# Alvin-Zeng/DRN

Hardware: AMD Instinct MI355X
Metric: clips/sec fwd+bwd (BxT=256x4096 C3D feats) (higher is better)
Workload: dtype bf16; 1 GPU; Charades-STA-shaped C3D features, T=256, D=4096, batch 32/GPU, stage-1 losses; step = fwd+bwd+grad all-reduce+clip(0.5)+Adam; global_batch=32, T=256, D=4096, parallelism=dp1

## Files before the change

drn_amd/csrc/lstm.hip:

```cpp
#include <type_traits>
#include "common.h"
#include "../../include/drn_hip.h"

#define LSTM_THREADS 256
#define MAX_BT 4

__device__ __forceinline__ float sigmoidf_(float x) { return 1.f / (1.f + expf(-x)); }

struct LstmFwdArgs {
  const float* xproj;
  const void* Whh[2];
  float* hseq;
  _Float16* hseq16;
  float* cseq;
  float* gates;
  float* out;
  float* hprev_t;
  float* qvec;
  const float* b_ih[2];
  const float* b_hh[2];
  const long long* lengths;
  int B, L, H, s;
};

// ... 17 lines not shown
#pragma unroll
    for (int g = 0; g < 4; ++g) {
      e_x[g] = A.xproj[(((long)t * B + bq) * 2 + dir) * 4 * H + g * H + e_j];
      e_bi[g] = A.b_ih[dir][g * H + e_j];
      e_bh[g] = A.b_hh[dir][g * H + e_j];
    }
    const long sp = ((long)(dir * (L + 1) + (s > 0 ? s : 1)) * B + bq) * H + e_j;
    e_cp = A.cseq[sp];
    e_hp = A.hseq[sp];
    e_len = A.lengths[bq];
    if (s == 0) { e_cp = 0.f; e_hp = 0.f; }
  }
  if (s > 0) {
    const int kq = H / 4;
    const int col = l & 15;
    const long wrow = (long)((col & 3) * H + j0 + (col >> 2)) * H;
    if constexpr (std::is_same<WT, float>::value) {
      const float* W = (const float*)A.Whh[dir];
      const int kc = (l >> 4) * 4;
      for (int k0 = w * kq; k0 < (w + 1) * kq; k0 += 16 * KU) {
        f32x4 a[KU][MT], b[KU];
#pragma unroll
        for (int u = 0; u < KU; ++u) {
          const int k = k0 + u * 16 + kc;
          b[u] = *(const f32x4*)(W + wrow + k);
#pragma unroll
          for (int mt = 0; mt < MT; ++mt) {
            const int bb = mt * 16 + col;
            a[u][mt] = *(const f32x4*)(hprev + (long)(bb < B ? bb : 0) * H + k);
            if (bb >= B) a[u][mt] = (f32x4){0.f, 0.f, 0.f, 0.f};
          }
        }
#pragma unroll
        for (int u = 0; u < KU; ++u)
#pragma unroll
          for (int e = 0; e < 4; ++e)
#pragma unroll
            for (int mt = 0; mt < MT; ++mt) acc[mt] = __builtin_amdgcn_mfma_f32_16x16x4f32(a[u][mt][e], b[u][e], acc[mt], 0, 0, 0);
      }
    } else if constexpr (std::is_same<WT, _Float16>::value) {
      typedef _Float16 f16x8 __attribute__((ext_vector_type(8)));
      const float* W = (const float*)A.Whh[dir];
      const _Float16* h16 = A.hseq16 + ((long)(dir * (L + 1) + s) * B) * H;
      const int kc = (l >> 4) * 8;
      for (int k0 = w * kq; k0 < (w + 1) * kq; k0 += 32 * KU) {
        f16x8 a[KU][MT];
        f32x4 blo[KU], bhi[KU];
#pragma unroll
        for (int u = 0; u < KU; ++u) {
          const int k = k0 + u * 32 + kc;
          blo[u] = *(const f32x4*)(W + wrow + k);
          bhi[u] = *(const f32x4*)(W + wrow + k + 4);
#pragma unroll
          for (int mt = 0; mt < MT; ++mt) {
            const int bb = mt * 16 + col;
            a[u][mt] = *(const f16x8*)(h16 + (long)(bb < B ? bb : 0) * H + k);
            if (bb >= B)
#pragma unroll
              for (int e = 0; e < 8; ++e) a[u][mt][e] = (_Float16)0.f;
          }
        }
#pragma unroll
        for (int u = 0; u < KU; ++u) {
          f16x8 bv;
#pragma unroll
          for (int e = 0; e < 4; ++e) { bv[e] = (_Float16)blo[u][e]; bv[4 + e] = (_Float16)bhi[u][e]; }
#pragma unroll
          for (int mt = 0; mt < MT; ++mt) acc[mt] = __builtin_amdgcn_mfma_f32_16x16x32_f16(a[u][mt], bv, acc[mt], 0, 0, 0);
        }
      }
    }
  }
#pragma unroll
  for (int mt = 0; mt < MT; ++mt)
#pragma unroll
    for (int r = 0; r < 4; ++r) red[w][mt][l][r] = acc[mt][r];
  __syncthreads();
  if (!e_own) return;
  {
    const int bb = e_bb, j = e_j;
    const int mt = bb >> 4, r16 = bb & 15, ln = (r16 >> 2) * 16 + (threadIdx.x & 3) * 4, rg = r16 & 3;
    float pre[4];
#pragma unroll
    for (int g = 0; g < 4; ++g) {
      const float v = red[0][mt][ln + g][rg] + red[1][mt][ln + g][rg] + red[2][mt][ln + g][rg] + red[3][mt][ln + g][rg];
      pre[g] = v + e_x[g] + e_bi[g] + e_bh[g];
    }
    const float ig = sigmoidf_(pre[0]), fg = sigmoidf_(pre[1]), gg = tanhf(pre[2]), og = sigmoidf_(pre[3]);
    const long st_new = ((long)(dir * (L + 1) + s + 1) * B + bb) * H + j;
    const float cp = e_cp, hp = e_hp;
    const float cn = fg * cp + ig * gg;
    const float hn = og * tanhf(cn);
    const bool valid = t < e_len;
    A.cseq[st_new] = valid ? cn : cp;
    A.hseq[st_new] = valid ? hn : hp;
    if (A.hseq16) A.hseq16[st_new] = (_Float16)(valid ? hn : hp);
    float* gs = A.gates + (((long)t * B + bb) * 2 + dir) * 4 * H + j;
    gs[0] = ig; gs[H] = fg; gs[2 * H] = gg; gs[3 * H] = og;
    A.hprev_t[(((long)t * B + bb) * 2 + dir) * H + j] = hp;
    A.out[((long)bb * L + t) * 2 * H + dir * H + j] = valid ? hn : 0.f;
    if (A.qvec) {
      float* qv = A.qvec + (long)bb * 4 * H + dir * H + j;
      if (t == 0) qv[0] = valid ? hn : 0.f;
      if (t == e_len - 1) qv[2 * H] = hn;
    }
  }
}

template <typename WT, int MT>
static void lstm_fwd_launch(const LstmFwdArgs& A, hipStream_t stream) {
  dim3 grid(A.H / 4, 2);
  const int per = std::is_same<WT, float>::value ? 16 : 32;
  const int it = A.H / 4 / per;
  if (it % 8 == 0 && std::is_same<WT, float>::value) lstm_step_fwd_kernel<WT, MT, 8><<<grid, LSTM_THREADS, 0, stream>>>(A);
  else if (it % 4 == 0) lstm_step_fwd_kernel<WT, MT, 4><<<grid, LSTM_THREADS, 0, stream>>>(A);
  else if (it % 2 == 0) lstm_step_fwd_kernel<WT, MT, 2><<<grid, LSTM_THREADS, 0, stream>>>(A);
  else lstm_step_fwd_kernel<WT, MT, 1><<<grid, LSTM_THREADS, 0, stream>>>(A);
}

extern "C" int drn_lstm_step_fwd(const float* xproj, const void* Whh_f, const void* Whh_r, int w_dtype, const float* b_ih_f,
                                 const float* b_hh_f, const float* b_ih_r, const float* b_hh_r, float* hseq, float* cseq, float* gates,
                                 float* out, float* hprev_t, float* qvec, void* hseq16, const int64_t* lengths, int B, int L, int H, int s,
                                 void* stream_) {
  drn_clear_status();
  hipStream_t stream = (hipStream_t)stream_;
  DRN_CHECK_ARG(xproj && Whh_f && Whh_r && b_ih_f && b_hh_f && b_ih_r && b_hh_r && hseq && cseq && gates && out && hprev_t && lengths,
                "drn_lstm_step_fwd: null pointer");
  DRN_CHECK_ARG(B > 0 && B <= 16 * MAX_BT && L > 0 && H % 64 == 0 && s >= 0 && s < L, "drn_lstm_step_fwd: need B<=64, H%%64==0");
  DRN_CHECK_ARG(w_dtype == DRN_F32, "drn_lstm_step_fwd: W_hh is fp32 (low precision enters through hseq16)");
  LstmFwdArgs A;
  DRN_CHECK_ARG(!hseq16 || (w_dtype == DRN_F32 && H % 128 == 0), "drn_lstm_step_fwd: the fp16 state copy goes with fp32 weights and H %% 128 == 0");
  A.hseq16 = (_Float16*)hseq16;
  A.xproj = xproj; A.Whh[0] = Whh_f; A.Whh[1] = Whh_r; A.hseq = hseq; A.cseq = cseq; A.gates = gates; A.out = out;
  A.hprev_t = hprev_t; A.qvec = qvec; A.b_ih[0] = b_ih_f; A.b_hh[0] = b_hh_f; A.b_ih[1] = b_ih_r; A.b_hh[1] = b_hh_r;
  A.lengths = (const long long*)lengths; A.B = B; A.L = L; A.H = H; A.s = s;
  const int mt = cdiv(B, 16);
  if (hseq16) {
    if (mt == 1) lstm_fwd_launch<_Float16, 1>(A, stream); else if (mt == 2) lstm_fwd_launch<_Float16, 2>(A, stream);
    else if (mt == 3) lstm_fwd_launch<_Float16, 3>(A, stream); else lstm_fwd_launch<_Float16, 4>(A, stream);
  } else {
    if (mt == 1) lstm_fwd_launch<float, 1>(A, stream); else if (mt == 2) lstm_fwd_launch<float, 2>(A, stream);
    else if (mt == 3) lstm_fwd_launch<float, 3>(A, stream); else lstm_fwd_launch<float, 4>(A, stream);
  }
  return drn_launch_status("drn_lstm_step_fwd");
}

struct LstmSeqArgs {
  LstmFwdArgs f;
  unsigned long long* xch;
  unsigned* counter;
};
static __device__ int g_lstm_seq_timeouts;

template <int MT, int KU>
__global__ __launch_bounds__(LSTM_THREADS) void lstm_seq_fwd_kernel(const LstmSeqArgs S) {
  typedef _Float16 f16x8 __attribute__((ext_vector_type(8)));
  __shared__ float red[4][MT][64][4];
  __shared__ unsigned s_launch;
  const LstmFwdArgs& A = S.f;
  const int w = threadIdx.x >> 6, l = threadIdx.x & 63;
  const int dir = blockIdx.y, j0 = blockIdx.x * 4;
  const int B = A.B, L = A.L, H = A.H;
  if (threadIdx.x == 0) s_launch = __hip_atomic_fetch_add(S.counter, 1u, __ATOMIC_RELAXED, __HIP_MEMORY_SCOPE_AGENT) / (gridDim.x * gridDim.y) + 1u;
  const int e_bb = threadIdx.x >> 2, e_j = j0 + (threadIdx.x & 3);
  const bool e_own = e_bb < B;
  const int bq = e_own ? e_bb : 0;
  float e_bi[4], e_bh[4];
#pragma unroll
  for (int g = 0; g < 4; ++g) {
    e_bi[g] = A.b_ih[dir][g * H + e_j];
    e_bh[g] = A.b_hh[dir][g * H + e_j];
  }
  const long long e_len = A.lengths[bq];
  float e_cp = 0.f, e_hp = 0.f;
  const int kq = H / 4, col = l & 15, kc = (l >> 4) * 8;
  const long wrow = (long)((col & 3) * H + j0 + (col >> 2)) * H;
  const float* W = (const float*)A.Whh[dir];
  __syncthreads();
  const unsigned long long tagm = (s_launch & 1u) ? 0x4000400040004000ull : 0ull;
  const long long t0 = wall_clock64();
  const bool w_resident = kq == 32 * KU;
  f16x8 wv[KU];
  if (w_resident) {
#pragma unroll
    for (int u = 0; u < KU; ++u) {
      const int k = w * kq + u * 32 + kc;
      const f32x4 lo = *(const f32x4*)(W + wrow + k), hi = *(const f32x4*)(W + wrow + k + 4);
#pragma unroll
      for (int e = 0; e < 4; ++e) { wv[u][e] = (_Float16)lo[e]; wv[u][4 + e] = (_Float16)hi[e]; }
    }
  }
  for (int s = 0; s < L; ++s) {
    const int t = dir == 0 ? s : L - 1 - s;
    float e_x[4];
#pragma unroll
    for (int g = 0; g < 4; ++g) e_x[g] = A.xproj[(((long)t * B + bq) * 2 + dir) * 4 * H + g * H + e_j];
    f32x4 acc[MT];
#pragma unroll
    for (int mt = 0; mt < MT; ++mt) acc[mt] = (f32x4){0.f, 0.f, 0.f, 0.f};
    if (s > 0) {
      const unsigned long long* hx = S.xch + ((long)(dir * L + s - 1) * B) * (H / 4);
      if (w == 0) {
        bool ready = false;
        for (;;) {
          if (!ready) {
            ready = true;
            for (int p = l; p < H / 4; p += 64)
              ready = ready && ((__hip_atomic_load(hx + p, __ATOMIC_RELAXED, __HIP_MEMORY_SCOPE_AGENT) & 0x4000400040004000ull) == tagm);
          }
          if (__builtin_amdgcn_ballot_w64(!ready) == 0) break;
          __builtin_amdgcn_s_sleep(4);
          if (wall_clock64() - t0 > 200000000LL) break;
        }
      }
      __syncthreads();
      for (int k0 = w * kq; k0 < (w + 1) * kq; k0 += 32 * KU) {
        unsigned long long alo[KU][MT], ahi[KU][MT];
        f32x4 blo[KU], bhi[KU];
#pragma unroll
        for (int u = 0; u < KU; ++u) {
          const int k = k0 + u * 32 + kc;
          if (!w_resident) {
            blo[u] = *(const f32x4*)(W + wrow + k);
            bhi[u] = *(const f32x4*)(W + wrow + k + 4);
          }
#pragma unroll
          for (int mt = 0; mt < MT; ++mt) {
            const int bb = mt * 16 + col;
            const unsigned long long* q = hx + (long)(bb < B ? bb : 0) * (H / 4) + (k >> 2);
            alo[u][mt] = __hip_atomic_load(q, __ATOMIC_RELAXED, __HIP_MEMORY_SCOPE_AGENT);
            ahi[u][mt] = __hip_atomic_load(q + 1, __ATOMIC_RELAXED, __HIP_MEMORY_SCOPE_AGENT);
          }
        }
#pragma unroll
        for (int u = 0; u < KU; ++u) {
          f16x8 bv;
          if (w_resident) bv = wv[u];
          else
#pragma unroll
            for (int e = 0; e < 4; ++e) { bv[e] = (_Float16)blo[u][e]; bv[4 + e] = (_Float16)bhi[u][e]; }
#pragma unroll
          for (int mt = 0; mt < MT; ++mt) {
            const int bb = mt * 16 + col;
            const unsigned long long* q = S.xch + ((long)(dir * L + s - 1) * B + (bb < B ? bb : 0)) * (H / 4) + ((k0 + u * 32 + kc) >> 2);
            while ((alo[u][mt] & 0x4000400040004000ull) != tagm || (ahi[u][mt] & 0x4000400040004000ull) != tagm) {
              __builtin_amdgcn_s_sleep(2);
              if (wall_clock64() - t0 > 200000000LL) {
                __hip_atomic_fetch_add(&g_lstm_seq_timeouts, 1, __ATOMIC_RELAXED, __HIP_MEMORY_SCOPE_AGENT);
                break;
              }
              alo[u][mt] = __hip_atomic_load(q, __ATOMIC_RELAXED, __HIP_MEMORY_SCOPE_AGENT);
              ahi[u][mt] = __hip_atomic_load(q + 1, __ATOMIC_RELAXED, __HIP_MEMORY_SCOPE_AGENT);
            }
            const unsigned long long lo = alo[u][mt] & ~0x4000400040004000ull, hi = ahi[u][mt] & ~0x4000400040004000ull;
            typedef unsigned long long u64x2 __attribute__((ext_vector_type(2)));
            f16x8 av = __builtin_bit_cast(f16x8, (u64x2){lo, hi});
            if (bb >= B)
#pragma unroll
              for (int e = 0; e < 8; ++e) av[e] = (_Float16)0.f;
            acc[mt] = __builtin_amdgcn_mfma_f32_16x16x32_f16(av, bv, acc[mt], 0, 0, 0);
          }
        }
      }
    }
#pragma unroll
    for (int mt = 0; mt < MT; ++mt)
#pragma unroll
      for (int r = 0; r < 4; ++r) red[w][mt][l][r] = acc[mt][r];
    __syncthreads();
    float h_new = 0.f;
    if (e_own) {
      const int bb = e_bb, j = e_j;
      const int mt = bb >> 4, r16 = bb & 15, ln = (r16 >> 2) * 16 + (threadIdx.x & 3) * 4, rg = r16 & 3;
      float pre[4];
#pragma unroll
      for (int g = 0; g < 4; ++g) {
        const float v = red[0][mt][ln + g][rg] + red[1][mt][ln + g][rg] + red[2][mt][ln + g][rg] + red[3][mt][ln + g][rg];
        pre[g] = v + e_x[g] + e_bi[g] + e_bh[g];
      }
      const float ig = sigmoidf_(pre[0]), fg = sigmoidf_(pre[1]), gg = tanhf(pre[2]), og = sigmoidf_(pre[3]);
      const long st_new = ((long)(dir * (L + 1) + s + 1) * B + bb) * H + j;
      const float cp = e_cp, hp = e_hp;
      const float cn = fg * cp + ig * gg;
      const float hn = og * tanhf(cn);
      const bool valid = t < e_len;
      e_cp = valid ? cn : cp;
      e_hp = valid ? hn : hp;
      h_new = e_hp;
      if (s + 1 < L) {
        const unsigned hb = (unsigned)__builtin_bit_cast(unsigned short, (_Float16)h_new);
        const unsigned h1 = (unsigned)__shfl_down((int)hb, 1, 64), h2 = (unsigned)__shfl_down((int)hb, 2, 64), h3 = (unsigned)__shfl_down((int)hb, 3, 64);
        if ((threadIdx.x & 3) == 0) {
          const unsigned long long word = ((unsigned long long)hb | ((unsigned long long)h1 << 16) | ((unsigned long long)h2 << 32) | ((unsigned long long)h3 << 48)) | tagm;
          __hip_atomic_store(S.xch + ((long)(dir * L + s) * B + e_bb) * (H / 4) + (j0 >> 2), word, __ATOMIC_RELAXED, __HIP_MEMORY_SCOPE_AGENT);
        }
      }
      A.cseq[st_new] = e_cp;
      A.hseq[st_new] = e_hp;
      float* gs = A.gates + (((long)t * B + bb) * 2 + dir) * 4 * H + j;
      gs[0] = ig; gs[H] = fg; gs[2 * H] = gg; gs[3 * H] = og;
      A.hprev_t[(((long)t * B + bb) * 2 + dir) * H + j] = hp;
      A.out[((long)bb * L + t) * 2 * H + dir * H + j] = valid ? hn : 0.f;
      if (A.qvec) {
        float* qv = A.qvec + (long)bb * 4 * H + dir * H + j;
        if (t == 0) qv[0] = valid ? hn : 0.f;
        if (t == e_len - 1) qv[2 * H] = hn;
      }
    }
    __syncthreads();
  }
}

static int lstm_seq_capacity(const void* kernel) {
  int dev = 0, per_cu = 0, cus = 0;
  if (hipGetDevice(&dev) != hipSuccess) return 0;
  if (hipDeviceGetAttribute(&cus, hipDeviceAttributeMultiprocessorCount, dev) != hipSuccess) return 0;
  if (hipOccupancyMaxActiveBlocksPerMultiprocessor(&per_cu, kernel, LSTM_THREADS, 0) != hipSuccess) return 0;
  hipFuncAttributes fa;
  if (hipFuncGetAttributes(&fa, kernel) != hipSuccess || fa.localSizeBytes > 0) return 0;
  return per_cu * cus;
}

extern "C" int64_t drn_lstm_seq_fwd_ws_bytes(int B, int L, int H) { return 64 + (int64_t)2 * L * B * (H / 4) * 8; }

extern "C" int drn_lstm_seq_fwd(const float* xproj, const void* Whh_f, const void* Whh_r, const float* b_ih_f, const float* b_hh_f,
                                const float* b_ih_r, const float* b_hh_r, float* hseq, float* cseq, float* gates, float* out, float* hprev_t,
                                float* qvec, void* xch_ws, int64_t ws_bytes, const int64_t* lengths, int B, int L, int H, void* stream_) {
  drn_clear_status();
  hipStream_t stream = (hipStream_t)stream_;
  DRN_CHECK_ARG(xproj && Whh_f && Whh_r && b_ih_f && b_hh_f && b_ih_r && b_hh_r && hseq && cseq && gates && out && hprev_t && lengths && xch_ws,
                "drn_lstm_seq_fwd: null pointer");
  DRN_CHECK_ARG(B > 0 && B <= 16 * MAX_BT && L > 0 && H % 128 == 0, "drn_lstm_seq_fwd: need B <= 64, H %% 128 == 0");
  DRN_CHECK_ARG(((uintptr_t)xch_ws & 63) == 0 && ws_bytes >= drn_lstm_seq_fwd_ws_bytes(B, L, H), "drn_lstm_seq_fwd: workspace too small or misaligned");
  LstmSeqArgs S;
  LstmFwdArgs& A = S.f;
  A.hseq16 = nullptr;
  A.xproj = xproj; A.Whh[0] = Whh_f; A.Whh[1] = Whh_r; A.hseq = hseq; A.cseq = cseq; A.gates = gates; A.out = out;
  A.hprev_t = hprev_t; A.qvec = qvec; A.b_ih[0] = b_ih_f; A.b_hh[0] = b_hh_f; A.b_ih[1] = b_ih_r; A.b_hh[1] = b_hh_r;
  A.lengths = (const long long*)lengths; A.B = B; A.L = L; A.H = H; A.s = 0;
  S.counter = (unsigned*)xch_ws;
  S.xch = (unsigned long long*)((char*)xch_ws + 64);
  const int mt = cdiv(B, 16), it = H / 4 / 32;
  const dim3 grid(H / 4, 2);
  const int total = (H / 4) * 2;
#define SEQ_CASE(MTV, KUV) do { \
    static int cap = 0; \
    if (!cap) cap = lstm_seq_capacity((const void*)lstm_seq_fwd_kernel<MTV, KUV>); \
    if (total > cap) { drn_set_error("drn_lstm_seq_fwd: %d workgroups exceed the %d the chip holds at once", total, cap); return DRN_ERR_UNSUPPORTED; } \
    lstm_seq_fwd_kernel<MTV, KUV><<<grid, LSTM_THREADS, 0, stream>>>(S); } while (0)
#define SEQ_MT(KUV) do { if (mt == 1) SEQ_CASE(1, KUV); else if (mt == 2) SEQ_CASE(2, KUV); else if (mt == 3) SEQ_CASE(3, KUV); else SEQ_CASE(4, KUV); } while (0)
  if (it % 4 == 0) SEQ_MT(4); else if (it % 2 == 0) SEQ_MT(2); else SEQ_MT(1);
#undef SEQ_MT
#undef SEQ_CASE
  return drn_launch_status("drn_lstm_seq_fwd");
}

extern "C" int drn_lstm_seq_fwd_timeouts(int reset) {
  int v = 0;
  if (hipMemcpyFromSymbol(&v, HIP_SYMBOL(g_lstm_seq_timeouts), sizeof(int)) != hipSuccess) return -1;
  if (reset && v) {
    const int z = 0;
    (void)hipMemcpyToSymbol(HIP_SYMBOL(g_lstm_seq_timeouts), &z, sizeof(int));
  }
  return v;
}

struct LstmBwdArgs {
  const float* dout;
  const float* gates;
  const float* cseq;
  const void* WhhT[2];
  float* dgates;
  float* dc;
  float* dh_pass;
  bf16_t* dgates16;
  const float* dqvec;
  const long long* lengths;
  int B, L, H, s;
};

struct LstmCellIn {
  float dout, dcn, ig, fg, gg, og, cn, cp;
  bool valid;
};
__device__ __forceinline__ LstmCellIn lstm_cell_bwd_load(const LstmBwdArgs& A, int dir, int bb, int j, int s) {
  const int B = A.B, L = A.L, H = A.H;
  const int t = dir == 0 ? s : L - 1 - s;
  LstmCellIn c;
  const long long len = A.lengths[bb];
  c.valid = t < len;
  const long sidx = ((long)dir * B + bb) * H + j;
  c.dout = A.dout[((long)bb * L + t) * 2 * H + dir * H + j];
  if (A.dqvec) {
    const float* dq = A.dqvec + (long)bb * 4 * H + dir * H + j;
    const float d0 = dq[0], d1 = dq[2 * H];
    if (t == 0) c.dout += d0;
    if (t == len - 1) c.dout += d1;
  }
  c.dcn = s == L - 1 ? 0.f : A.dc[sidx];
  const float* gs = A.gates + (((long)t * B + bb) * 2 + dir) * 4 * H + j;
  c.ig = gs[0]; c.fg = gs[H]; c.gg = gs[2 * H]; c.og = gs[3 * H];
  c.cn = A.cseq[((long)(dir * (L + 1) + s + 1) * B + bb) * H + j];
  c.cp = A.cseq[((long)(dir * (L + 1) + (s > 0 ? s : 1)) * B + bb) * H + j];
  if (s == 0) c.cp = 0.f;
  return c;
}
__device__ __forceinline__ void lstm_cell_bwd_apply(const LstmBwdArgs& A, const LstmCellIn& c, int dir, int bb, int j, int s, float dh_in) {
#pragma clang fp contract(off)
  const int B = A.B, L = A.L, H = A.H;
  const int t = dir == 0 ? s : L - 1 - s;
  const long sidx = ((long)dir * B + bb) * H + j;
  const long gidx = (((long)t * B + bb) * 2 + dir) * 4 * H + j;
  float* dg = A.dgates + gidx;
  const float dh = dh_in + (c.valid ? c.dout : 0.f);
  const float dcn = c.dcn;
  float d0 = 0.f, d1 = 0.f, d2 = 0.f, d3 = 0.f;
  if (c.valid) {
    const float ig = c.ig, fg = c.fg, gg = c.gg, og = c.og, cn = c.cn, cp = c.cp;
    const float tc = tanhf(cn);
    const float dcv = dcn + dh * og * (1.f - tc * tc);
    d0 = dcv * gg * ig * (1.f - ig);
    d1 = dcv * cp * fg * (1.f - fg);
    d2 = dcv * ig * (1.f - gg * gg);
    d3 = dh * tc * og * (1.f - og);
    A.dc[sidx] = dcv * fg;
    A.dh_pass[sidx] = 0.f;
  } else {
    A.dc[sidx] = dcn;
    A.dh_pass[sidx] = dh;
  }
  dg[0] = d0; dg[H] = d1; dg[2 * H] = d2; dg[3 * H] = d3;
  if (A.dgates16) {
    bf16_t* dg16 = A.dgates16 + gidx;
    dg16[0] = (bf16_t)d0; dg16[H] = (bf16_t)d1; dg16[2 * H] = (bf16_t)d2; dg16[3 * H] = (bf16_t)d3;
  }
}
__device__ __forceinline__ void lstm_cell_bwd(const LstmBwdArgs& A, int dir, int bb, int j, int s, float dh_in) {
  const LstmCellIn c = lstm_cell_bwd_load(A, dir, bb, j, s);
  lstm_cell_bwd_apply(A, c, dir, bb, j, s, dh_in);
}

__global__ void lstm_bwd_first_kernel(const LstmBwdArgs A) {
  const int B = A.B, H = A.H;
  const int total = 2 * B * H;
  for (int idx = blockIdx.x * blockDim.x + threadIdx.x; idx < total; idx += gridDim.x * blockDim.x)
    lstm_cell_bwd(A, idx / (H * B), (idx / H) % B, idx % H, A.L - 1, 0.f);
}

template <typename WT, int KU>
__global__ __launch_bounds__(LSTM_THREADS) void lstm_step_bwd_kernel(const LstmBwdArgs A) {
  __shared__ float red[4][64][4];
  const int w = threadIdx.x >> 6, l = threadIdx.x & 63;
  const int dir = blockIdx.y, k0 = blockIdx.x * 16, bt = blockIdx.z;
  const int B = A.B, L = A.L, H = A.H, s = A.s;
  const int K = 4 * H, kq = K / 4;
  const int t = dir == 0 ? s : L - 1 - s;
  const float* dg = A.dgates + ((long)t * B * 2 + dir) * K;
  f32x4 acc = (f32x4){0.f, 0.f, 0.f, 0.f};
  const int row = l & 15;
  const int bb_a = bt * 16 + row;
  const int e_bb = bt * 16 + (l >> 4) * 4 + w, e_k = k0 + (l & 15);
  const bool e_own = e_bb < B;
  const LstmCellIn e_c = lstm_cell_bwd_load(A, dir, e_own ? e_bb : 0, e_k, s - 1);
  const float e_dhp = A.dh_pass[((long)dir * B + (e_own ? e_bb : 0)) * H + e_k];
  const float* arow = dg + (long)(bb_a < B ? bb_a : 0) * 2 * K;
  if constexpr (std::is_same<WT, float>::value) {
    const float* WT_ = (const float*)A.WhhT[dir];
    const int rc = (l >> 4) * 4;
    for (int r0 = w * kq; r0 < (w + 1) * kq; r0 += 16 * KU) {
      f32x4 a[KU], b[KU];
#pragma unroll
      for (int u = 0; u < KU; ++u) {
        const int r = r0 + u * 16 + rc;
        a[u] = *(const f32x4*)(arow + r);
        if (bb_a >= B) a[u] = (f32x4){0.f, 0.f, 0.f, 0.f};
        b[u] = *(const f32x4*)(WT_ + (long)(k0 + row) * K + r);
      }
#pragma unroll
      for (int u = 0; u < KU; ++u)
#pragma unroll
        for (int e = 0; e < 4; ++e) acc = __builtin_amdgcn_mfma_f32_16x16x4f32(a[u][e], b[u][e], acc, 0, 0, 0);
    }
  } else {
    const bf16_t* WT_ = (const bf16_t*)A.WhhT[dir];
    const int rc = (l >> 4) * 8;
    if (A.dgates16) {
      const bf16_t* arow16 = A.dgates16 + ((long)t * B * 2 + dir) * K + (long)(bb_a < B ? bb_a : 0) * 2 * K;
      for (int r0 = w * kq; r0 < (w + 1) * kq; r0 += 32 * KU) {
        bf16x8 a[KU], b[KU];
#pragma unroll
        for (int u = 0; u < KU; ++u) {
          const int r = r0 + u * 32 + rc;
          a[u] = *(const bf16x8*)(arow16 + r);
          if (bb_a >= B)
#pragma unroll
            for (int e = 0; e < 8; ++e) a[u][e] = (bf16_t)0.f;
          b[u] = *(const bf16x8*)(WT_ + (long)(k0 + row) * K + r);
        }
#pragma unroll
        for (int u = 0; u < KU; ++u) acc = __builtin_amdgcn_mfma_f32_16x16x32_bf16(a[u], b[u], acc, 0, 0, 0);
      }
    } else
// ... 69 lines not shown
```

drn_amd/trainer.py:

```python
import contextlib
import functools
import os

import torch

from . import functional as DF
import numpy as np

from .metrics import results_entries, PostProcessRunner, results_entry, recall_from_first_hits


def stage_plan(model, stage, lr):
    dead = set(id(p) for p in model.unused_parameters()) if hasattr(model, "unused_parameters") else set()
    if stage == 1:
        for name, p in model.named_parameters():
            if "iou_scores" in name or "mix_fc" in name:
                p.requires_grad = False
        return [p for p in model.parameters() if p.requires_grad and id(p) not in dead], lr, 10, "sum"
    if stage == 2:
        head = model.fcos.head
        return list(head.iou_scores.parameters()) + list(head.mix_fc.parameters()), lr / 100, None, "loss_iou"
    if stage == 3:
        return [p for p in model.parameters() if id(p) not in dead], lr / 10000, None, "sum"
    raise ValueError("stage must be 1, 2 or 3")
# ... 187 lines not shown
                        self.reducer.rearm()
                    slot.graph.replay()
                    if getattr(slot, "acc_outside", False):
                        self._accumulate(select_loss(slot.out, self.which), slot.feats.size(0))
                    if not whole:
                        self._exchange_and_update()
                    out = slot.out
                else:
                    slot.seen += 1
                    out = self._fwd_bwd(slot.args)
                    self._exchange_and_update()
        cur.wait_stream(self.stream)
        return out

    def train_step(self, args):
        self.model.train()
        if self.graph:
            return self._graph_step(args)
        if self.fused:
            self.reducer.zero()
        _, loss_dict = self.model(*args)
        DF.backward(select_loss(loss_dict, self.which))
        if self.fused:
            self.reducer.finish()
            self.opt.step()
        else:
            if self.world_size > 1:
                self._average_grads()
            if self.clip is not None:
                torch.nn.utils.clip_grad_norm_(self.model.parameters(), self.clip)
            self.opt.step()
            self.opt.zero_grad()
        return loss_dict

    def _average_grads(self):
        import torch.distributed as td
        grads = [p.grad for p in self.model.parameters() if p.grad is not None]
        if not grads:
            return
        flat = torch._utils._flatten_dense_tensors(grads)
        td.all_reduce(flat)
        flat.div_(self.world_size)
        for g, r in zip(grads, torch._utils._unflatten_dense_tensors(flat, grads)):
            g.copy_(r)

    def train_epoch(self, loader, epoch=None):
        sampler = getattr(loader, "sampler", None)
        if epoch is not None and hasattr(sampler, "set_epoch"):
            sampler.set_epoch(epoch)
        n = 0
        if getattr(self, "_loss_acc", None) is None:
            self._loss_acc = torch.zeros((), dtype=torch.float32, device=getattr(self, "device", "cpu"))
        if getattr(self, "graph", False) and getattr(self, "prefetch", False):
            it = iter(loader)
            nxt = self._prefetch(next(it, None))
            with torch.cuda.stream(self.stream):
                self._loss_acc.zero_()
            while nxt is not None:
                cur_b = nxt
                nxt = self._prefetch(next(it, None))
                bs = cur_b.batch_size if isinstance(cur_b, _Preloaded) else cur_b[2].size(0)
                self.train_step(cur_b)
                n += bs
            torch.cuda.current_stream().wait_stream(self.stream)
            return self._epoch_result(n)
        with torch.cuda.stream(self.stream) if self.graph else contextlib.nullcontext():
            self._loss_acc.zero_()
        for batch in loader:
            if self.graph:
                names, pse, feats, gt, tok, qlen, nprops, nframes = batch
                args = (tok, qlen, feats, pse, gt, nprops, nframes)
            else:
                _, args = to_device(batch, self.device)
            bs = args[2].size(0)
            ld = self.train_step(args)
            if not self.graph:
                self._accumulate(select_loss(ld, self.which), bs)
            n += bs
        if self.graph:
            torch.cuda.current_stream().wait_stream(self.stream)
        return self._epoch_result(n)

    def _epoch_result(self, n):
        mean = float(self._loss_acc) / max(n, 1) if n else 0.0
        if getattr(getattr(self, "device", None), "type", "cpu") == "cuda":
            from . import ops
            ops.check_watchdogs()
        return mean

    def _prefetch(self, batch):
        if batch is None:
            return None
        names, pse, feats, gt, tok, qlen, nprops, nframes = batch
        if all(t.is_cuda for t in (tok, qlen, feats, pse, gt)):
            return (tok, qlen, feats, pse, gt, nprops, nframes)
        slot = self._slot_for(tok, feats, pse, gt, alternate=True)
        if slot is None:
            return (tok, qlen, feats, pse, gt, nprops, nframes)
        if self._copy_stream is None:
            self._copy_stream = torch.cuda.Stream(device=self.device)
        cs = self._copy_stream
        cs.wait_stream(torch.cuda.current_stream())
        with torch.cuda.stream(cs):
            slot.load(tok, qlen, feats, pse, gt)
            ev = torch.cuda.Event()
            ev.record(cs)
        for t in (tok, qlen, feats, pse, gt):
            if t.is_cuda:
                t.record_stream(cs)
        return _Preloaded(slot, ev, int(feats.size(0)))

    @torch.no_grad()
    def evaluate(self, loader, id2word=None, iou_topk=None, with_results=True, group=None):
        self.model.eval()
        import torch.distributed as td
        multi = td.is_available() and td.is_initialized() and td.get_world_size(group) > 1
        if multi:
            from .dist import sync_model_state
            sync_model_state(self.model, src=0, group=group, buffers_only=True)
        iou_topk = iou_topk or {"iou": [0.5], "topk": [1, 5]}
        results, total, n, hits = {}, None, 0, []
        selector = getattr(getattr(self.model, "fcos", None), "box_selector_test", None)
        head = getattr(getattr(self.model, "fcos", None), "head", None)
        one_class = head is None or head.cls_logits.weight.shape[0] == 1
        fast = (not with_results) and selector is not None and self.device.type == "cuda" and one_class
        fast0 = fast
        ious_dev = torch.tensor([float(x) for x in iou_topk["iou"]], dtype=torch.float64, device=self.device) if fast else None
        if fast:
            selector.device_only = True
        try:
            for batch in loader:
                host_tok, host_qlen, host_gt = batch[4], batch[5], batch[3]
                names, args = to_device(batch, self.device)
                boxes, loss_dict = self.model(*args)
                bs = args[2].size(0)
                lsum = select_loss(loss_dict, self.which).detach().reshape(-1)[0].float() * bs
                total = lsum if total is None else total + lsum
                n += bs
                if fast and not isinstance(boxes, list):
                    from . import ops
                    hits.append(ops.eval_recall(boxes.det, boxes.scores, boxes.counts, args[4].contiguous(), ious_dev,
                                                max(iou_topk["topk"])))
                    continue
                if fast:
                    raise RuntimeError("Trainer.evaluate: the post-processor returned host records in device-only mode")
                tokens, qlen, gts = host_tok.cpu(), host_qlen.cpu(), host_gt.cpu().numpy()
                queries = [" ".join(id2word[int(t)] if id2word else str(int(t)) for t in tokens[i, :int(qlen[i])]) for i in range(bs)]
                for name, entry in zip(names, results_entries(queries, gts, boxes)):
                    results.setdefault(name, []).append(entry)
        finally:
            if fast:
                selector.device_only = False
        total = float(total) if total is not None else 0.0
        if fast0:
            fh = torch.cat(hits).cpu().numpy() if hits else np.zeros((0, len(iou_topk["iou"])), dtype=np.int32)
            if multi:
                parts = [None] * td.get_world_size(group)
                td.all_gather_object(parts, ("hits", fh, total, n), group=group)
                assert all(p[0] == "hits" for p in parts), "ranks disagree on the evaluation path"
                fh = np.concatenate([p[1] for p in parts])
                total, n = sum(p[2] for p in parts), sum(p[3] for p in parts)
            return total / max(n, 1), iou_topk["topk"], recall_from_first_hits(fh, iou_topk["iou"], iou_topk["topk"]), None
        if multi:
            parts = [None] * td.get_world_size(group)
            td.all_gather_object(parts, ("records", results, total, n), group=group)
            assert all(p[0] == "records" for p in parts), "ranks disagree on the evaluation path"
            parts = [p[1:] for p in parts]
            results = {}
            for part, _, _ in parts:
                for vid, items in part.items():
                    results.setdefault(vid, []).extend(items)
            total, n = sum(p[1] for p in parts), sum(p[2] for p in parts)
        topks, accs = PostProcessRunner(results).run_evaluate(iou_topk_dict=iou_topk, temporal_nms=True)
        return total / max(n, 1), topks, accs, results

    @torch.no_grad()
    def predict(self, loader, top_k=5, nms_overlap=0.45, share_videos=True, id2word=None, fused=False, graph=False):
        from .grounding import Grounder, group_by_video
        was_training = self.model.training
        self.model.eval()
        grounder = Grounder(self.model, top_k=top_k, nms_overlap=nms_overlap, fused=fused, graph=graph)
        out = {}
        try:
            for batch in loader:
                names, pse, feats, _, tok, qlen = batch[:6]
                mv = lambda t: t.to(self.device, non_blocking=True)
                vid = None
                if share_videos:
                    unique, vid = group_by_video(names)
                    if len(unique) < len(names):
                        first = torch.tensor([names.index(u) for u in unique], dtype=torch.int64)
                        feats, pse = feats.index_select(0, first.to(feats.device)), pse.index_select(0, first.to(pse.device))
                    else:
                        vid = None
                moments = grounder.ground(mv(tok), mv(qlen), mv(feats), mv(pse), vid).tolist()
                tokens, lens = tok.cpu(), qlen.cpu()
                for i, name in enumerate(names):
                    query = " ".join(id2word[int(t)] if id2word else str(int(t)) for t in tokens[i, :int(lens[i])])
                    out.setdefault(name, []).append({"query": query, "moments": moments[i]})
        finally:
            self.model.train(was_training)
        return out

    def fit(self, train_loader, test_loader, n_epoch=None, eval_freq=1, snapshot_pref=None, dataset="Charades", id2word=None,
            start_epoch=0, rank=0):
        n_epoch = self.default_epochs if self.default_epochs is not None else n_epoch
        best1 = best5 = 0.0
        history = []
        for epoch in range(start_epoch, n_epoch):
            train_loss = self.train_epoch(train_loader, epoch)
            rec = {"epoch": epoch, "train_loss": train_loss}
            if (epoch + 1) % eval_freq == 0 or epoch == n_epoch - 1:
                val_loss, topks, accs, _ = self.evaluate(test_loader, id2word, with_results=False)
                top1, top5 = accs[0] * 100, accs[1] * 100
                rec.update(val_loss=val_loss, top1=top1, top5=top5)
                state = {"epoch": epoch + 1, "state_dict": checkpoint_state_dict(self.model), "loss": val_loss, "top1": top1,
                         "top5": top5}
                if snapshot_pref is not None and rank == 0:
                    if top1 > best1:
                        save_checkpoint(state, snapshot_pref, dataset, epoch, top1, top5)
                    if top5 > best5:
                        save_checkpoint(state, snapshot_pref, dataset, epoch, top1, top5)
                best1, best5 = max(best1, top1), max(best5, top5)
            history.append(rec)
        return history


    def fit_train_only(self, train_loader, n_epoch, start_epoch=0):
        n_epoch = self.default_epochs if self.default_epochs is not None else n_epoch
        return [{"epoch": e, "train_loss": self.train_epoch(train_loader, e)} for e in range(start_epoch, n_epoch)]


def checkpoint_state_dict(model):
    DF.flush_bn_counters()
    return {"module." + k: v for k, v in model.state_dict().items()}


def checkpoint_name(snapshot_pref, dataset, epoch, top1, top5):
    return "{}/model_{}_epoch{}_top1_{:.3f}_top5_{:.3f}_model_best.pth.tar".format(snapshot_pref, dataset, epoch, top1, top5)


def save_checkpoint(state, snapshot_pref, dataset, epoch, top1, top5):
    os.makedirs(snapshot_pref, exist_ok=True)
    path = checkpoint_name(snapshot_pref, dataset, epoch, top1, top5)
    torch.save(state, path)
    return path


def load_checkpoint(model, path, map_location="cpu"):
    ckpt = torch.load(path, map_location=map_location)
    own = model.state_dict()
    picked = {}
    for k, v in ckpt["state_dict"].items():
        k = k[len("module."):] if k.startswith("module.") else k
        if k in own:
            picked[k] = v
    own.update(picked)
    model.load_state_dict(own)
    DF.bump_weights_epoch([DF.store_of(next(model.parameters()))])
    return ckpt.get("epoch", 0), sorted(picked)


def init_glove(model, glove_weights):
    if glove_weights and os.path.exists(glove_weights):
        model.query_encoder.embedding.weight.data.copy_(torch.load(glove_weights))
        DF.bump_weights_epoch([DF.store_of(model.query_encoder.embedding.weight)])
        return True
    return False
```

Before: 17490 clips/s.

## Widen LSTM sequence workgroups to 16 hidden units with LDS-resident recurrent weights

The persistent LSTM forward kernel now has each workgroup own 16 hidden units instead of 4, which cuts the grid by four. Each workgroup caches its slice of W_hh as fp16 in dynamic LDS, and each wave computes four MFMA N-tiles per h fragment, so every exchanged h load is reused four times. The wave-0 pre-spin barrier is removed, the gate math is spread across lanes via shuffles, and the next step's xproj is prefetched. The trade-off is a large LDS footprint per workgroup and fewer workgroups for the cross-block h exchange. The trainer also adds a watchdog check after evaluation.

```diff
diff --git a/drn_amd/csrc/lstm.hip b/drn_amd/csrc/lstm.hip
--- a/drn_amd/csrc/lstm.hip
+++ b/drn_amd/csrc/lstm.hip
@@ -193,170 +193,203 @@
 };
 static __device__ int g_lstm_seq_timeouts;
 
+#define SEQ_TAG 0x4000400040004000ull
+#define SEQ_TIMEOUT 200000000LL
+
+static inline size_t lstm_seq_lds_bytes(int H, int mt) { return (size_t)128 * H + (size_t)16384 * mt; }
+
 template <int MT, int KU>
 __global__ __launch_bounds__(LSTM_THREADS) void lstm_seq_fwd_kernel(const LstmSeqArgs S) {
   typedef _Float16 f16x8 __attribute__((ext_vector_type(8)));
-  __shared__ float red[4][MT][64][4];
+  extern __shared__ __attribute__((aligned(16))) char smem[];
   __shared__ unsigned s_launch;
   const LstmFwdArgs& A = S.f;
   const int w = threadIdx.x >> 6, l = threadIdx.x & 63;
-  const int dir = blockIdx.y, j0 = blockIdx.x * 4;
+  const int dir = blockIdx.y, j0 = blockIdx.x * 16;
   const int B = A.B, L = A.L, H = A.H;
+  const int kq = H / 4, ki = kq / 32;
+  f16x8* wf = (f16x8*)smem + (size_t)w * ki * 256;
+  float* red = (float*)(smem + (size_t)128 * H);
   if (threadIdx.x == 0) s_launch = __hip_atomic_fetch_add(S.counter, 1u, __ATOMIC_RELAXED, __HIP_MEMORY_SCOPE_AGENT) / (gridDim.x * gridDim.y) + 1u;
-  const int e_bb = threadIdx.x >> 2, e_j = j0 + (threadIdx.x & 3);
-  const bool e_own = e_bb < B;
-  const int bq = e_own ? e_bb : 0;
+  const int q = l & 3, cu = (l >> 2) & 3, rg = l >> 4;
+  const int e_j = j0 + w * 4 + cu;
   float e_bi[4], e_bh[4];
 #pragma unroll
   for (int g = 0; g < 4; ++g) {
     e_bi[g] = A.b_ih[dir][g * H + e_j];
     e_bh[g] = A.b_hh[dir][g * H + e_j];
   }
-  const long long e_len = A.lengths[bq];
-  float e_cp = 0.f, e_hp = 0.f;
-  const int kq = H / 4, col = l & 15, kc = (l >> 4) * 8;
-  const long wrow = (long)((col & 3) * H + j0 + (col >> 2)) * H;
-  const float* W = (const float*)A.Whh[dir];
+  int e_bb[MT], e_bq[MT];
+  long long e_len[MT];
+  float e_cp[MT], e_hp[MT], e_x[MT][4];
+#pragma unroll
+  for (int mt = 0; mt < MT; ++mt) {
+    e_bb[mt] = mt * 16 + rg * 4 + q;
+    e_bq[mt] = e_bb[mt] < B ? e_bb[mt] : 0;
+    e_len[mt] = A.lengths[e_bq[mt]];
+    e_cp[mt] = 0.f; e_hp[mt] = 0.f;
+    const int t = dir == 0 ? 0 : L - 1;
+#pragma unroll
+    for (int g = 0; g < 4; ++g) e_x[mt][g] = A.xproj[(((long)t * B + e_bq[mt]) * 2 + dir) * 4 * H + g * H + e_j];
+  }
+  const int col = l & 15, kc = (l >> 4) * 8;
+  {
+    const float* W = (const float*)A.Whh[dir];
+    for (int f0 = 0; f0 < ki * 4; f0 += 4) {
+      f32x4 lo[4], hi[4];
+#pragma unroll
+      for (int i = 0; i < 4; ++i) {
+        const int f = f0 + i, u = f >> 2, n = f & 3;
+        const float* p = W + (long)((col & 3) * H + j0 + n * 4 + (col >> 2)) * H + w * kq + u * 32 + kc;
+        lo[i] = *(const f32x4*)p;
+        hi[i] = *(const f32x4*)(p + 4);
+      }
+#pragma unroll
+      for (int i = 0; i < 4; ++i) {
+        f16x8 v;
+#pragma unroll
+        for (int e = 0; e < 4; ++e) { v[e] = (_Float16)lo[i][e]; v[4 + e] = (_Float16)hi[i][e]; }
+        wf[(f0 + i) * 64 + l] = v;
+      }
+    }
+  }
   __syncthreads();
-  const unsigned long long tagm = (s_launch & 1u) ? 0x4000400040004000ull : 0ull;
+  const unsigned long long tagm = (s_launch & 1u) ? SEQ_TAG : 0ull;
   const long long t0 = wall_clock64();
-  const bool w_resident = kq == 32 * KU;
-  f16x8 wv[KU];
-  if (w_resident) {
-#pragma unroll
-    for (int u = 0; u < KU; ++u) {
-      const int k = w * kq + u * 32 + kc;
-      const f32x4 lo = *(const f32x4*)(W + wrow + k), hi = *(const f32x4*)(W + wrow + k + 4);
-#pragma unroll
-      for (int e = 0; e < 4; ++e) { wv[u][e] = (_Float16)lo[e]; wv[u][4 + e] = (_Float16)hi[e]; }
-    }
-  }
   for (int s = 0; s < L; ++s) {
     const int t = dir == 0 ? s : L - 1 - s;
-    float e_x[4];
-#pragma unroll
-    for (int g = 0; g < 4; ++g) e_x[g] = A.xproj[(((long)t * B + bq) * 2 + dir) * 4 * H + g * H + e_j];
-    f32x4 acc[MT];
-#pragma unroll
-    for (int mt = 0; mt < MT; ++mt) acc[mt] = (f32x4){0.f, 0.f, 0.f, 0.f};
+    f32x4 x[MT];
+#pragma unroll
+    for (int mt = 0; mt < MT; ++mt) x[mt] = (f32x4){0.f, 0.f, 0.f, 0.f};
     if (s > 0) {
+      f32x4 acc[MT][4];
+#pragma unroll
+      for (int mt = 0; mt < MT; ++mt)
+#pragma unroll
+        for (int n = 0; n < 4; ++n) acc[mt][n] = (f32x4){0.f, 0.f, 0.f, 0.f};
       const unsigned long long* hx = S.xch + ((long)(dir * L + s - 1) * B) * (H / 4);
-      if (w == 0) {
-        bool ready = false;
-        for (;;) {
-          if (!ready) {
-            ready = true;
-            for (int p = l; p < H / 4; p += 64)
-              ready = ready && ((__hip_atomic_load(hx + p, __ATOMIC_RELAXED, __HIP_MEMORY_SCOPE_AGENT) & 0x4000400040004000ull) == tagm);
-          }
-          if (__builtin_amdgcn_ballot_w64(!ready) == 0) break;
-          __builtin_amdgcn_s_sleep(4);
-          if (wall_clock64() - t0 > 200000000LL) break;
-        }
-      }
-      __syncthreads();
-      for (int k0 = w * kq; k0 < (w + 1) * kq; k0 += 32 * KU) {
+      for (int i0 = 0; i0 < ki; i0 += KU) {
         unsigned long long alo[KU][MT], ahi[KU][MT];
-        f32x4 blo[KU], bhi[KU];
-#pragma unroll
-        for (int u = 0; u < KU; ++u) {
-          const int k = k0 + u * 32 + kc;
-          if (!w_resident) {
-            blo[u] = *(const f32x4*)(W + wrow + k);
-            bhi[u] = *(const f32x4*)(W + wrow + k + 4);
-          }
+#pragma unroll
+        for (int u = 0; u < KU; ++u)
 #pragma unroll
           for (int mt = 0; mt < MT; ++mt) {
             const int bb = mt * 16 + col;
-            const unsigned long long* q = hx + (long)(bb < B ? bb : 0) * (H / 4) + (k >> 2);
-            alo[u][mt] = __hip_atomic_load(q, __ATOMIC_RELAXED, __HIP_MEMORY_SCOPE_AGENT);
-            ahi[u][mt] = __hip_atomic_load(q + 1, __ATOMIC_RELAXED, __HIP_MEMORY_SCOPE_AGENT);
+            const unsigned long long* p = hx + (long)(bb < B ? bb : 0) * (H / 4) + ((w * kq + (i0 + u) * 32 + kc) >> 2);
+            alo[u][mt] = __hip_atomic_load(p, __ATOMIC_RELAXED, __HIP_MEMORY_SCOPE_AGENT);
+            ahi[u][mt] = __hip_atomic_load(p + 1, __ATOMIC_RELAXED, __HIP_MEMORY_SCOPE_AGENT);
           }
-        }
 #pragma unroll
         for (int u = 0; u < KU; ++u) {
-          f16x8 bv;
-          if (w_resident) bv = wv[u];
-          else
-#pragma unroll
-            for (int e = 0; e < 4; ++e) { bv[e] = (_Float16)blo[u][e]; bv[4 + e] = (_Float16)bhi[u][e]; }
+          f16x8 bv[4];
+#pragma unroll
+          for (int n = 0; n < 4; ++n) bv[n] = wf[((i0 + u) * 4 + n) * 64 + l];
 #pragma unroll
           for (int mt = 0; mt < MT; ++mt) {
             const int bb = mt * 16 + col;
-            const unsigned long long* q = S.xch + ((long)(dir * L + s - 1) * B + (bb < B ? bb : 0)) * (H / 4) + ((k0 + u * 32 + kc) >> 2);
-            while ((alo[u][mt] & 0x4000400040004000ull) != tagm || (ahi[u][mt] & 0x4000400040004000ull) != tagm) {
+            const unsigned long long* p = hx + (long)(bb < B ? bb : 0) * (H / 4) + ((w * kq + (i0 + u) * 32 + kc) >> 2);
+            while ((alo[u][mt] & SEQ_TAG) != tagm || (ahi[u][mt] & SEQ_TAG) != tagm) {
               __builtin_amdgcn_s_sleep(2);
-              if (wall_clock64() - t0 > 200000000LL) {
+              if (wall_clock64() - t0 > SEQ_TIMEOUT) {
                 __hip_atomic_fetch_add(&g_lstm_seq_timeouts, 1, __ATOMIC_RELAXED, __HIP_MEMORY_SCOPE_AGENT);
                 break;
               }
-              alo[u][mt] = __hip_atomic_load(q, __ATOMIC_RELAXED, __HIP_MEMORY_SCOPE_AGENT);
-              ahi[u][mt] = __hip_atomic_load(q + 1, __ATOMIC_RELAXED, __HIP_MEMORY_SCOPE_AGENT);
+              alo[u][mt] = __hip_atomic_load(p, __ATOMIC_RELAXED, __HIP_MEMORY_SCOPE_AGENT);
+              ahi[u][mt] = __hip_atomic_load(p + 1, __ATOMIC_RELAXED, __HIP_MEMORY_SCOPE_AGENT);
             }
-            const unsigned long long lo = alo[u][mt] & ~0x4000400040004000ull, hi = ahi[u][mt] & ~0x4000400040004000ull;
             typedef unsigned long long u64x2 __attribute__((ext_vector_type(2)));
-            f16x8 av = __builtin_bit_cast(f16x8, (u64x2){lo, hi});
-            if (bb >= B)
-#pragma unroll
-              for (int e = 0; e < 8; ++e) av[e] = (_Float16)0.f;
-            acc[mt] = __builtin_amdgcn_mfma_f32_16x16x32_f16(av, bv, acc[mt], 0, 0, 0);
+            const f16x8 av = __builtin_bit_cast(f16x8, (u64x2){alo[u][mt] & ~SEQ_TAG, ahi[u][mt] & ~SEQ_TAG});
+#pragma unroll
+            for (int n = 0; n < 4; ++n) acc[mt][n] = __builtin_amdgcn_mfma_f32_16x16x32_f16(av, bv[n], acc[mt][n], 0, 0, 0);
           }
         }
       }
-    }
-#pragma unroll
-    for (int mt = 0; mt < MT; ++mt)
-#pragma unroll
-      for (int r = 0; r < 4; ++r) red[w][mt][l][r] = acc[mt][r];
-    __syncthreads();
-    float h_new = 0.f;
-    if (e_own) {
-      const int bb = e_bb, j = e_j;
-      const int mt = bb >> 4, r16 = bb & 15, ln = (r16 >> 2) * 16 + (threadIdx.x & 3) * 4, rg = r16 & 3;
+#pragma unroll
+      for (int mt = 0; mt < MT; ++mt)
+#pragma unroll
+        for (int n = 0; n < 4; ++n) *(f32x4*)(red + ((((w * MT + mt) * 4 + n) * 64 + l) * 4)) = acc[mt][n];
+      __syncthreads();
+#pragma unroll
+      for (int mt = 0; mt < MT; ++mt) {
+        const f32x4 r0 = *(const f32x4*)(red + ((((0 * MT + mt) * 4 + w) * 64 + l) * 4)), r1 = *(const f32x4*)(red + ((((1 * MT + mt) * 4 + w) * 64 + l) * 4)),
+                    r2 = *(const f32x4*)(red + ((((2 * MT + mt) * 4 + w) * 64 + l) * 4)), r3 = *(const f32x4*)(red + ((((3 * MT + mt) * 4 + w) * 64 + l) * 4));
+#pragma unroll
+        for (int r = 0; r < 4; ++r) x[mt][r] = r0[r] + r1[r] + r2[r] + r3[r];
+      }
+    }
+    unsigned hb[MT];
+    float pg[MT][4], p_hp[MT], p_out[MT], p_hn[MT];
+    bool p_valid[MT];
+#pragma unroll
+    for (int mt = 0; mt < MT; ++mt) {
+      float v4[4];
+#pragma unroll
+      for (int g = 0; g < 4; ++g) {
+        const int src = (l & ~3) + g;
+        const float y0 = __shfl(x[mt][0], src, 64), y1 = __shfl(x[mt][1], src, 64), y2 = __shfl(x[mt][2], src, 64), y3 = __shfl(x[mt][3], src, 64);
+        v4[g] = q == 0 ? y0 : q == 1 ? y1 : q == 2 ? y2 : y3;
+      }
       float pre[4];
 #pragma unroll
       for (int g = 0; g < 4; ++g) {
-        const float v = red[0][mt][ln + g][rg] + red[1][mt][ln + g][rg] + red[2][mt][ln + g][rg] + red[3][mt][ln + g][rg];
-        pre[g] = v + e_x[g] + e_bi[g] + e_bh[g];
+        const float v = v4[g];
+        pre[g] = v + e_x[mt][g] + e_bi[g] + e_bh[g];
       }
       const float ig = sigmoidf_(pre[0]), fg = sigmoidf_(pre[1]), gg = tanhf(pre[2]), og = sigmoidf_(pre[3]);
-      const long st_new = ((long)(dir * (L + 1) + s + 1) * B + bb) * H + j;
-      const float cp = e_cp, hp = e_hp;
+      const float cp = e_cp[mt], hp = e_hp[mt];
       const float cn = fg * cp + ig * gg;
       const float hn = og * tanhf(cn);
-      const bool valid = t < e_len;
-      e_cp = valid ? cn : cp;
-      e_hp = valid ? hn : hp;
-      h_new = e_hp;
-      if (s + 1 < L) {
-        const unsigned hb = (unsigned)__builtin_bit_cast(unsigned short, (_Float16)h_new);
-        const unsigned h1 = (unsigned)__shfl_down((int)hb, 1, 64), h2 = (unsigned)__shfl_down((int)hb, 2, 64), h3 = (unsigned)__shfl_down((int)hb, 3, 64);
-        if ((threadIdx.x & 3) == 0) {
-          const unsigned long long word = ((unsigned long long)hb | ((unsigned long long)h1 << 16) | ((unsigned long long)h2 << 32) | ((unsigned long long)h3 << 48)) | tagm;
-          __hip_atomic_store(S.xch + ((long)(dir * L + s) * B + e_bb) * (H / 4) + (j0 >> 2), word, __ATOMIC_RELAXED, __HIP_MEMORY_SCOPE_AGENT);
+      const bool valid = t < e_len[mt];
+      e_cp[mt] = valid ? cn : cp;
+      e_hp[mt] = valid ? hn : hp;
+      pg[mt][0] = ig; pg[mt][1] = fg; pg[mt][2] = gg; pg[mt][3] = og;
+      p_hp[mt] = hp; p_out[mt] = valid ? hn : 0.f; p_hn[mt] = hn; p_valid[mt] = valid;
+      hb[mt] = (unsigned)__builtin_bit_cast(unsigned short, (_Float16)e_hp[mt]);
+    }
+    if (s + 1 < L) {
+#pragma unroll
+      for (int mt = 0; mt < MT; ++mt) {
+        const int base = l & ~12;
+        const unsigned h1 = (unsigned)__shfl((int)hb[mt], base | 4, 64), h2 = (unsigned)__shfl((int)hb[mt], base | 8, 64), h3 = (unsigned)__shfl((int)hb[mt], base | 12, 64);
+        if (cu == 0 && e_bb[mt] < B) {
+          const unsigned long long word = ((unsigned long long)hb[mt] | ((unsigned long long)h1 << 16) | ((unsigned long long)h2 << 32) | ((unsigned long long)h3 << 48)) | tagm;
+          __hip_atomic_store(S.xch + ((long)(dir * L + s) * B + e_bb[mt]) * (H / 4) + ((j0 + w * 4) >> 2), word, __ATOMIC_RELAXED, __HIP_MEMORY_SCOPE_AGENT);
         }
       }
-      A.cseq[st_new] = e_cp;
-      A.hseq[st_new] = e_hp;
+      const int tn = dir == 0 ? s + 1 : L - 2 - s;
+#pragma unroll
+      for (int mt = 0; mt < MT; ++mt)
+#pragma unroll
+        for (int g = 0; g < 4; ++g) e_x[mt][g] = A.xproj[(((long)tn * B + e_bq[mt]) * 2 + dir) * 4 * H + g * H + e_j];
+    }
+#pragma unroll
+    for (int mt = 0; mt < MT; ++mt) {
+      if (e_bb[mt] >= B) continue;
+      const int bb = e_bb[mt], j = e_j;
+      const long st_new = ((long)(dir * (L + 1) + s + 1) * B + bb) * H + j;
+      A.cseq[st_new] = e_cp[mt];
+      A.hseq[st_new] = e_hp[mt];
       float* gs = A.gates + (((long)t * B + bb) * 2 + dir) * 4 * H + j;
-      gs[0] = ig; gs[H] = fg; gs[2 * H] = gg; gs[3 * H] = og;
-      A.hprev_t[(((long)t * B + bb) * 2 + dir) * H + j] = hp;
-      A.out[((long)bb * L + t) * 2 * H + dir * H + j] = valid ? hn : 0.f;
+      gs[0] = pg[mt][0]; gs[H] = pg[mt][1]; gs[2 * H] = pg[mt][2]; gs[3 * H] = pg[mt][3];
+      A.hprev_t[(((long)t * B + bb) * 2 + dir) * H + j] = p_hp[mt];
+      A.out[((long)bb * L + t) * 2 * H + dir * H + j] = p_out[mt];
       if (A.qvec) {
         float* qv = A.qvec + (long)bb * 4 * H + dir * H + j;
-        if (t == 0) qv[0] = valid ? hn : 0.f;
-        if (t == e_len - 1) qv[2 * H] = hn;
+        if (t == 0) qv[0] = p_out[mt];
+        if (t == e_len[mt] - 1) qv[2 * H] = p_hn[mt];
       }
     }
     __syncthreads();
   }
 }
 
-static int lstm_seq_capacity(const void* kernel) {
+static int lstm_seq_capacity(const void* kernel, size_t lds) {
   int dev = 0, per_cu = 0, cus = 0;
   if (hipGetDevice(&dev) != hipSuccess) return 0;
   if (hipDeviceGetAttribute(&cus, hipDeviceAttributeMultiprocessorCount, dev) != hipSuccess) return 0;
-  if (hipOccupancyMaxActiveBlocksPerMultiprocessor(&per_cu, kernel, LSTM_THREADS, 0) != hipSuccess) return 0;
+  if (lds + 64 > 163840) return 0;
+  if (hipFuncSetAttribute(kernel, hipFuncAttributeMaxDynamicSharedMemorySize, (int)lds) != hipSuccess) { (void)hipGetLastError(); return 0; }
+  if (hipOccupancyMaxActiveBlocksPerMultiprocessor(&per_cu, kernel, LSTM_THREADS, lds) != hipSuccess) { (void)hipGetLastError(); return 0; }
   hipFuncAttributes fa;
   if (hipFuncGetAttributes(&fa, kernel) != hipSuccess || fa.localSizeBytes > 0) return 0;
   return per_cu * cus;
@@ -371,7 +404,7 @@
   hipStream_t stream = (hipStream_t)stream_;
   DRN_CHECK_ARG(xproj && Whh_f && Whh_r && b_ih_f && b_hh_f && b_ih_r && b_hh_r && hseq && cseq && gates && out && hprev_t && lengths && xch_ws,
                 "drn_lstm_seq_fwd: null pointer");
-  DRN_CHECK_ARG(B > 0 && B <= 16 * MAX_BT && L > 0 && H % 128 == 0, "drn_lstm_seq_fwd: need B <= 64, H %% 128 == 0");
+  DRN_CHECK_ARG(B > 0 && B <= 16 * MAX_BT && L > 0 && H > 0 && H % 128 == 0, "drn_lstm_seq_fwd: need B <= 64, H %% 128 == 0");
   DRN_CHECK_ARG(((uintptr_t)xch_ws & 63) == 0 && ws_bytes >= drn_lstm_seq_fwd_ws_bytes(B, L, H), "drn_lstm_seq_fwd: workspace too small or misaligned");
   LstmSeqArgs S;
   LstmFwdArgs& A = S.f;
@@ -382,13 +415,14 @@
   S.counter = (unsigned*)xch_ws;
   S.xch = (unsigned long long*)((char*)xch_ws + 64);
   const int mt = cdiv(B, 16), it = H / 4 / 32;
-  const dim3 grid(H / 4, 2);
-  const int total = (H / 4) * 2;
+  const dim3 grid(H / 16, 2);
+  const int total = (H / 16) * 2;
+  const size_t lds = lstm_seq_lds_bytes(H, mt);
 #define SEQ_CASE(MTV, KUV) do { \
-    static int cap = 0; \
-    if (!cap) cap = lstm_seq_capacity((const void*)lstm_seq_fwd_kernel<MTV, KUV>); \
-    if (total > cap) { drn_set_error("drn_lstm_seq_fwd: %d workgroups exceed the %d the chip holds at once", total, cap); return DRN_ERR_UNSUPPORTED; } \
-    lstm_seq_fwd_kernel<MTV, KUV><<<grid, LSTM_THREADS, 0, stream>>>(S); } while (0)
+    static int cap = 0, cap_h = 0; \
+    if (cap_h != H) { cap = lstm_seq_capacity((const void*)lstm_seq_fwd_kernel<MTV, KUV>, lds); cap_h = H; } \
+    if (total > cap) { drn_set_error("drn_lstm_seq_fwd: %d workgroups of %zu LDS bytes exceed the %d the chip holds at once", total, lds, cap); return DRN_ERR_UNSUPPORTED; } \
+    lstm_seq_fwd_kernel<MTV, KUV><<<grid, LSTM_THREADS, lds, stream>>>(S); } while (0)
 #define SEQ_MT(KUV) do { if (mt == 1) SEQ_CASE(1, KUV); else if (mt == 2) SEQ_CASE(2, KUV); else if (mt == 3) SEQ_CASE(3, KUV); else SEQ_CASE(4, KUV); } while (0)
   if (it % 4 == 0) SEQ_MT(4); else if (it % 2 == 0) SEQ_MT(2); else SEQ_MT(1);
 #undef SEQ_MT
diff --git a/drn_amd/trainer.py b/drn_amd/trainer.py
--- a/drn_amd/trainer.py
+++ b/drn_amd/trainer.py
@@ -363,6 +363,9 @@
             if fast:
                 selector.device_only = False
         total = float(total) if total is not None else 0.0
+        if self.device.type == "cuda":
+            from . import ops
+            ops.check_watchdogs()
         if fast0:
             fh = torch.cat(hits).cpu().numpy() if hits else np.zeros((0, len(iou_topk["iou"])), dtype=np.int32)
             if multi:
```

Result: no change. 17500 clips/s, median of 2 (+0.0%).
